# utcsilab/score-based-channels

Hardware: AMD Instinct MI355X
Metric: channels/s full ALD inference, CDL-C Nt64xNr16 (higher is better)
Workload: dtype f16x2 (every fp32 operand as two fp16 terms of a power-of-two-scaled value = 22-bit significand, hh + hl + lh on the fp16 matrix cores, fp32 accumulate; fp32-class by the gate tests/test_gpu_parity.py::test_f16x2_is_fp32_class and held to every reference golden at the north_star tolerance; unconditi

## Files before the change

### score_based_channels_amd/csrc/conv_down.hip

```cpp
#include <stdlib.h>
#include <string.h>
#include <type_traits>
#include "conv_common.h"

namespace sbc {

typedef float f32x4v __attribute__((ext_vector_type(4)));

struct DownParams {
    const float* __restrict__ a;
    const float* __restrict__ x;
    float* __restrict__ out;
    const float* __restrict__ stats;
    const uint4* __restrict__ w4;
    const uint4* __restrict__ w2;
    const float* __restrict__ bias;
    const float* __restrict__ bias2;
    unsigned* __restrict__ range_flag;
    float* __restrict__ calib;
    int B, H;
};

template <int B_, int E_, class F>
__device__ __forceinline__ void down_static_for(F&& f) {
    if constexpr (B_ < E_) {
        f(std::integral_constant<int, B_>{});
        down_static_for<B_ + 1, E_>(f);
    }
}

template <int CIN, int COUT, int W>
__global__ __launch_bounds__(256, 2) void conv_down_kernel(DownParams p) {
    constexpr int WO = W / 2, R = 8, NR = 2 * R + 2;
    constexpr int RP = W == 16 ? 12 : 6;
    constexpr int CG = CIN / 8, KH = CIN / 32, C4 = CIN / 4, NCB = COUT / 16;
    constexpr int NU = R * WO / 16;
    constexpr int RPU = 16 / WO;
    constexpr int PS = (2 * NR * RP * 16 + 255) / 256 * 256;
    constexpr int TERM = CG * PS;
    static_assert(NCB == 4, "four waves, one 16-output-channel block each");
    static_assert((W == 16 && CIN == 32) || (W == 8 && CIN == 64), "res2.0 (32 -> 64 at 16-pixel rows) and res3.0 (64 -> 64 at 8)");
    extern __shared__ __attribute__((aligned(256))) unsigned char smem[];

    const int tid = threadIdx.x, lane = tid & 63;
    const int cb = __builtin_amdgcn_readfirstlane(tid >> 6);
    const int kq = lane >> 4, n = lane & 15;
    const int H = p.H, HO = H / 2;
    const int tiles = HO / R;
    const int s = blockIdx.x / tiles, y0 = (blockIdx.x - s * tiles) * R;
    const int r_in0 = 2 * y0 - 1;

    const int wl_base = (((kq >> 1) * (COUT / 32) + (cb >> 1)) * 2) * 64 + (16 * (cb & 1) + n) + 32 * (kq & 1);
    constexpr int WD = 4;
    uint4 wr[WD][2];
    auto ldw = [&](const uint4* __restrict__ w, int tap, int kh, int slot) {
        const int idx = wl_base + ((tap * (CIN / 16) + 2 * kh) * (COUT / 32) * 2) * 64;
        wr[slot][0] = w[idx];
        wr[slot][1] = w[idx + 64];
    };
    const float4 tr4 = f16x2_trailer(reinterpret_cast<const float4*>(p.w4), 16 * (CIN / 16) * (COUT / 32) * 2);
    const float4 tr2 = f16x2_trailer(reinterpret_cast<const float4*>(p.w2), 4 * (CIN / 16) * (COUT / 32) * 2);
    const float scale_m = __builtin_bit_cast(float, __builtin_amdgcn_readfirstlane(__builtin_bit_cast(int, tr4.x)));
    const float scale_s = __builtin_bit_cast(float, __builtin_amdgcn_readfirstlane(__builtin_bit_cast(int, tr2.x)));
    const float descale_m = tr4.y, descale_s = tr2.y;
    const bool elu_acc = __builtin_amdgcn_readfirstlane(__builtin_bit_cast(int, tr4.w)) != 0;
    unsigned rbits = 0;

    const int c4 = tid % C4;
    constexpr int CPR = W * C4;
    auto plane_dst = [&](int prow, int col) {
        return smem + (c4 >> 1) * PS + (((col & 1) * NR + prow) * RP + (col >> 1) + (col & 1)) * 16 + (c4 & 1) * 8;
    };
    for (int i = tid; i < 2 * TERM / 16; i += 256) *reinterpret_cast<uint4*>(smem + i * 16) = make_uint4(0, 0, 0, 0);

    constexpr int NQA = NR * CPR / 256, NQX = 2 * R * CPR / 256;
    static_assert(NR * CPR % 256 == 0 && 2 * R * CPR % 256 == 0, "whole rounds of chunks");
    float4 va[NQA];
    const float* a_base = p.a + (size_t)s * H * W * CIN;
#pragma unroll
    for (int k = 0; k < NQA; ++k) {
        const int q = k * 256 + tid, prow = q / CPR;
        const int r = r_in0 + prow;
        va[k] = make_float4(0.f, 0.f, 0.f, 0.f);
        if (r >= 0 && r < H) va[k] = *reinterpret_cast<const float4*>(a_base + (size_t)r * W * CIN + (q - prow * CPR) * 4);
    }
    const float* st = p.stats + (size_t)s * 3 * CIN + c4 * 4;
    const float4 mu = *reinterpret_cast<const float4*>(st), sc = *reinterpret_cast<const float4*>(st + CIN),
                 sh = *reinterpret_cast<const float4*>(st + 2 * CIN);
    ldw(p.w4, 0, 0, 0);
    ldw(p.w4, 1 / KH, 1 % KH, 1);
    ldw(p.w4, 2 / KH, 2 % KH, 2);
    __syncthreads();
    float ta = 0.f;
#pragma unroll
    for (int k = 0; k < NQA; ++k) {
        const int q = k * 256 + tid, prow = q / CPR, col = (q - prow * CPR) / C4;
        const int r = r_in0 + prow;
        if (r < 0 || r >= H) continue;
        float4 v = va[k];
        v.x = fmaf(v.x - mu.x, sc.x, sh.x); v.y = fmaf(v.y - mu.y, sc.y, sh.y);
        v.z = fmaf(v.z - mu.z, sc.z, sh.z); v.w = fmaf(v.w - mu.w, sc.w, sh.w);
        v = elu4(v, elu_acc);
        StageScale ss{scale_m, ta};
        scale_track(v, &ss);
        ta = ss.amax;
        uint2 h, l;
        split_f16x2(v, scale_m, h, l);
        unsigned char* dst = plane_dst(prow, col);
        *reinterpret_cast<uint2*>(dst) = h;
        *reinterpret_cast<uint2*>(dst + TERM) = l;
    }
    pair_range_tile(ta, scale_m, rbits, p.calib);
    float4 vx[NQX];
    const float* x_base = p.x + ((size_t)s * H + 2 * y0) * W * CIN;
#pragma unroll
    for (int k = 0; k < NQX; ++k) vx[k] = *reinterpret_cast<const float4*>(x_base + (size_t)(k * 256 + tid) * 4);
    lds_barrier();

    const int yl0 = n / WO, xo = n % WO;
    const int rd_base = kq * PS + ((2 * yl0) * RP + xo) * 16;
    f32x4v accm[NU], accs[NU];
    auto kloop = [&](auto mainc, const uint4* __restrict__ w, f32x4v* acc) {
        constexpr bool MAIN = decltype(mainc)::value;
        constexpr int KT = MAIN ? 4 : 2, NS = KT * KT * KH;
        down_static_for<0, NS>([&](auto sc_) {
            constexpr int s_ = decltype(sc_)::value;
            constexpr int tap = s_ / KH, kh = s_ % KH, tp = tap / KT, tq = tap % KT;
            if constexpr (s_ + WD - 1 < NS) ldw(w, (s_ + WD - 1) / KH, (s_ + WD - 1) % KH, (s_ + WD - 1) % WD);
            const f16x8 wh = __builtin_bit_cast(f16x8, wr[s_ % WD][0]);
            const f16x8 wl = __builtin_bit_cast(f16x8, wr[s_ % WD][1]);
            constexpr int prow = MAIN ? tp : tp + 1, q = MAIN ? tq : tq + 1;
            constexpr int off = (4 * kh) * PS + ((((q + 1) & 1) * NR + prow) * RP + (q >> 1)) * 16;
            f16x8 xh[NU], xl[NU];
#pragma unroll
            for (int u = 0; u < NU; ++u) {
                xh[u] = *reinterpret_cast<const f16x8*>(smem + rd_base + off + (2 * u * RPU * RP) * 16);
                xl[u] = *reinterpret_cast<const f16x8*>(smem + rd_base + off + (2 * u * RPU * RP) * 16 + TERM);
            }
#pragma unroll
            for (int u = 0; u < NU; ++u) {
                const f32x4v z = s_ == 0 ? f32x4v{0.f, 0.f, 0.f, 0.f} : acc[u];
                acc[u] = __builtin_amdgcn_mfma_f32_16x16x32_f16(wh, xl[u], z, 0, 0, 0);
            }
#pragma unroll
            for (int u = 0; u < NU; ++u) acc[u] = __builtin_amdgcn_mfma_f32_16x16x32_f16(wl, xh[u], acc[u], 0, 0, 0);
#pragma unroll
            for (int u = 0; u < NU; ++u) acc[u] = __builtin_amdgcn_mfma_f32_16x16x32_f16(wh, xh[u], acc[u], 0, 0, 0);
            __builtin_amdgcn_sched_barrier(0);
        });
    };
    kloop(std::true_type{}, p.w4, accm);

    ldw(p.w2, 0, 0, 0);
    ldw(p.w2, 1 / KH, 1 % KH, 1);
    ldw(p.w2, 2 / KH, 2 % KH, 2);
    float tb = 0.f;
    uint2 xh_[NQX], xl_[NQX];
#pragma unroll
    for (int k = 0; k < NQX; ++k) {
        StageScale ss{scale_s, tb};
        scale_track(vx[k], &ss);
        tb = ss.amax;
        split_f16x2(vx[k], scale_s, xh_[k], xl_[k]);
    }
    pair_range_tile(tb, scale_s, rbits, p.calib ? p.calib + 1 : nullptr);
    lds_barrier();
#pragma unroll
    for (int k = 0; k < NQX; ++k) {
        const int q = k * 256 + tid, prow = q / CPR, col = (q - prow * CPR) / C4;
        unsigned char* dst = plane_dst(prow + 1, col);
        *reinterpret_cast<uint2*>(dst) = xh_[k];
        *reinterpret_cast<uint2*>(dst + TERM) = xl_[k];
    }
    lds_barrier();
    kloop(std::false_type{}, p.w2, accs);

    const int ch0 = 16 * cb + 4 * kq;
    const f32x4v b2 = *reinterpret_cast<const f32x4v*>(p.bias + ch0), bs = *reinterpret_cast<const f32x4v*>(p.bias2 + ch0);
#pragma unroll
    for (int u = 0; u < NU; ++u) {
        float4 o;
        o.x = fmaf(accs[u][0], descale_s, bs[0]) + fmaf(accm[u][0], descale_m, b2[0]);
        o.y = fmaf(accs[u][1], descale_s, bs[1]) + fmaf(accm[u][1], descale_m, b2[1]);
        o.z = fmaf(accs[u][2], descale_s, bs[2]) + fmaf(accm[u][2], descale_m, b2[2]);
        o.w = fmaf(accs[u][3], descale_s, bs[3]) + fmaf(accm[u][3], descale_m, b2[3]);
        const int y = y0 + u * RPU + yl0;
        st_out(p.out + (((size_t)s * HO + y) * WO + xo) * COUT + ch0, o);
    }
    if (rbits && lane == 0) atomicOr(p.range_flag, rbits);
}

template <int CIN, int COUT, int W>
static int launch_down_t(const DownParams& p, hipStream_t stream, bool dry) {
    constexpr int NR = 18, RP = W == 16 ? 12 : 6;
    constexpr int PS = (2 * NR * RP * 16 + 255) / 256 * 256;
    constexpr int LDS = 2 * (CIN / 8) * PS;
    auto kern = conv_down_kernel<CIN, COUT, W>;
    { const int rc = ensure_dyn_lds(reinterpret_cast<const void*>(kern), LDS); if (rc) return rc; }
    if (dry) return SBC_OK;
    hipLaunchKernelGGL(kern, dim3(p.B * (p.H / 2 / 8)), dim3(256), LDS, stream, p);
    SBC_CHECK_HIP(hipGetLastError());
    return SBC_OK;
}

int launch_conv_down(const sbc_op& op, hipStream_t stream, bool dry) {
    SBC_REQUIRE(op.in && op.out && op.res1 && op.stats && op.weight_split && op.weight2_split && op.bias && op.bias2,
                "conv_down: in / res1 / out / stats / weight_split / weight2_split / bias / bias2 must be set");
    SBC_REQUIRE((op.W == 16 && op.cin == 32 && op.cout == 64) || (op.W == 8 && op.cin == 64 && op.cout == 64),
                "conv_down: 32 -> 64 channels at 16-pixel rows or 64 -> 64 at 8 (got %d -> %d, W = %d)", op.cin, op.cout, op.W);
    SBC_REQUIRE(op.H % 16 == 0 && op.H >= 16, "conv_down: H = %d must be a multiple of 16 (tiles of 8 pooled rows)", op.H);
    SBC_REQUIRE((op.flags & SBC_CONV_F16X2) && !(op.flags & SBC_CONV_F16W), "conv_down: SBC_CONV_F16X2 only (the weight forms it reads)");
    SBC_REQUIRE(op.out != op.in && op.out != op.res1, "conv_down: out must not alias its inputs");
    SBC_REQUIRE(op.B > 0 && (long)op.B * op.H * op.W * op.cin <= 0x7fffffffL, "conv_down: bad batch %d", op.B);
    DownParams p;
    memset(&p, 0, sizeof(p));
    p.a = (const float*)op.in; p.x = (const float*)op.res1; p.out = (float*)op.out; p.stats = (const float*)op.stats;
    p.w4 = (const uint4*)op.weight_split; p.w2 = (const uint4*)op.weight2_split;
    p.bias = (const float*)op.bias; p.bias2 = (const float*)op.bias2;
    p.calib = (float*)op.calib;
    p.B = op.B; p.H = op.H;
    unsigned* flag = nullptr;
    { const int rc = range_flag_ptr(&flag); if (rc) return rc; }
    p.range_flag = flag;
    return op.W == 16 ? launch_down_t<32, 64, 16>(p, stream, dry) : launch_down_t<64, 64, 8>(p, stream, dry);
}

}
```

Baseline: 56.86.

## Make conv_down persistent with XCD-aware tiling and cross-tile prefetch

The down-sampling conv kernel now launches a persistent grid of about two workgroups per CU, grouped per XCD. Each workgroup walks a contiguous range of tiles and prefetches the next tile's activations, residual and stats while the current tile's MFMA loops run. The shortcut weights are held in registers for the whole kernel, and the LDS zero-fill happens once instead of per tile. This cuts launch/tail imbalance and global-load latency between tiles, at the cost of more register pressure, extra barriers per tile, and a hipDeviceGetAttribute query on every launch.

New measurement: 56.84 (median of 2 runs). No clear change (-0.0%).

```diff
diff --git a/score_based_channels_amd/csrc/conv_down.hip b/score_based_channels_amd/csrc/conv_down.hip
--- a/score_based_channels_amd/csrc/conv_down.hip
+++ b/score_based_channels_amd/csrc/conv_down.hip
@@ -19,6 +19,7 @@
     unsigned* __restrict__ range_flag;
     float* __restrict__ calib;
     int B, H;
+    int ntiles, tiles_per_xcd, wgs_per_xcd;
 };
 
 template <int B_, int E_, class F>
@@ -47,16 +48,25 @@
     const int kq = lane >> 4, n = lane & 15;
     const int H = p.H, HO = H / 2;
     const int tiles = HO / R;
-    const int s = blockIdx.x / tiles, y0 = (blockIdx.x - s * tiles) * R;
-    const int r_in0 = 2 * y0 - 1;
-
-    const int wl_base = (((kq >> 1) * (COUT / 32) + (cb >> 1)) * 2) * 64 + (16 * (cb & 1) + n) + 32 * (kq & 1);
+
+    const int xcd = blockIdx.x & 7, jw = blockIdx.x >> 3;
+    const int t_begin = xcd * p.tiles_per_xcd;
+    const int cnt = max(min(t_begin + p.tiles_per_xcd, p.ntiles) - t_begin, 0);
+    const int t0 = t_begin + jw * cnt / p.wgs_per_xcd, t1 = t_begin + (jw + 1) * cnt / p.wgs_per_xcd;
+    if (t0 >= t1) return;
+
+    auto opaque = [](int v) { asm volatile("" : "+v"(v)); return v; };
+    auto wl_base = [&](int l) { return ((((l >> 4) >> 1) * (COUT / 32) + (cb >> 1)) * 2) * 64 + (16 * (cb & 1) + (l & 15)) + 32 * ((l >> 4) & 1); };
     constexpr int WD = 4;
     uint4 wr[WD][2];
-    auto ldw = [&](const uint4* __restrict__ w, int tap, int kh, int slot) {
-        const int idx = wl_base + ((tap * (CIN / 16) + 2 * kh) * (COUT / 32) * 2) * 64;
-        wr[slot][0] = w[idx];
-        wr[slot][1] = w[idx + 64];
+    auto ldw = [&](const uint4* __restrict__ w, int wb, int tap, int kh, uint4* dst) {
+        const int idx = wb + ((tap * (CIN / 16) + 2 * kh) * (COUT / 32) * 2) * 64;
+        dst[0] = w[idx];
+        dst[1] = w[idx + 64];
+    };
+    auto ring_start = [&](const uint4* __restrict__ w) {
+        const int wb = wl_base(opaque(lane));
+        down_static_for<0, WD - 1>([&](auto sc_) { ldw(w, wb, decltype(sc_)::value / KH, decltype(sc_)::value % KH, wr[decltype(sc_)::value]); });
     };
     const float4 tr4 = f16x2_trailer(reinterpret_cast<const float4*>(p.w4), 16 * (CIN / 16) * (COUT / 32) * 2);
     const float4 tr2 = f16x2_trailer(reinterpret_cast<const float4*>(p.w2), 4 * (CIN / 16) * (COUT / 32) * 2);
@@ -65,70 +75,63 @@
     const float descale_m = tr4.y, descale_s = tr2.y;
     const bool elu_acc = __builtin_amdgcn_readfirstlane(__builtin_bit_cast(int, tr4.w)) != 0;
     unsigned rbits = 0;
-
-    const int c4 = tid % C4;
+    const int ch0 = 16 * cb + 4 * kq;
+    const f32x4v b2 = *reinterpret_cast<const f32x4v*>(p.bias + ch0), bs = *reinterpret_cast<const f32x4v*>(p.bias2 + ch0);
+    constexpr int NSS = 4 * KH;
+    uint4 ws[NSS][2];
+    down_static_for<0, NSS>([&](auto sc_) { ldw(p.w2, wl_base(lane), decltype(sc_)::value / KH, decltype(sc_)::value % KH, ws[decltype(sc_)::value]); });
+
     constexpr int CPR = W * C4;
-    auto plane_dst = [&](int prow, int col) {
+    auto plane_dst = [&](int tq, int prow, int col) {
+        const int c4 = tq % C4;
         return smem + (c4 >> 1) * PS + (((col & 1) * NR + prow) * RP + (col >> 1) + (col & 1)) * 16 + (c4 & 1) * 8;
     };
-    for (int i = tid; i < 2 * TERM / 16; i += 256) *reinterpret_cast<uint4*>(smem + i * 16) = make_uint4(0, 0, 0, 0);
-
     constexpr int NQA = NR * CPR / 256, NQX = 2 * R * CPR / 256;
     static_assert(NR * CPR % 256 == 0 && 2 * R * CPR % 256 == 0, "whole rounds of chunks");
-    float4 va[NQA];
-    const float* a_base = p.a + (size_t)s * H * W * CIN;
-#pragma unroll
-    for (int k = 0; k < NQA; ++k) {
-        const int q = k * 256 + tid, prow = q / CPR;
-        const int r = r_in0 + prow;
-        va[k] = make_float4(0.f, 0.f, 0.f, 0.f);
-        if (r >= 0 && r < H) va[k] = *reinterpret_cast<const float4*>(a_base + (size_t)r * W * CIN + (q - prow * CPR) * 4);
-    }
-    const float* st = p.stats + (size_t)s * 3 * CIN + c4 * 4;
-    const float4 mu = *reinterpret_cast<const float4*>(st), sc = *reinterpret_cast<const float4*>(st + CIN),
-                 sh = *reinterpret_cast<const float4*>(st + 2 * CIN);
-    ldw(p.w4, 0, 0, 0);
-    ldw(p.w4, 1 / KH, 1 % KH, 1);
-    ldw(p.w4, 2 / KH, 2 % KH, 2);
-    __syncthreads();
-    float ta = 0.f;
-#pragma unroll
-    for (int k = 0; k < NQA; ++k) {
-        const int q = k * 256 + tid, prow = q / CPR, col = (q - prow * CPR) / C4;
-        const int r = r_in0 + prow;
-        if (r < 0 || r >= H) continue;
-        float4 v = va[k];
-        v.x = fmaf(v.x - mu.x, sc.x, sh.x); v.y = fmaf(v.y - mu.y, sc.y, sh.y);
-        v.z = fmaf(v.z - mu.z, sc.z, sh.z); v.w = fmaf(v.w - mu.w, sc.w, sh.w);
-        v = elu4(v, elu_acc);
-        StageScale ss{scale_m, ta};
-        scale_track(v, &ss);
-        ta = ss.amax;
-        uint2 h, l;
-        split_f16x2(v, scale_m, h, l);
-        unsigned char* dst = plane_dst(prow, col);
-        *reinterpret_cast<uint2*>(dst) = h;
-        *reinterpret_cast<uint2*>(dst + TERM) = l;
-    }
-    pair_range_tile(ta, scale_m, rbits, p.calib);
-    float4 vx[NQX];
-    const float* x_base = p.x + ((size_t)s * H + 2 * y0) * W * CIN;
-#pragma unroll
-    for (int k = 0; k < NQX; ++k) vx[k] = *reinterpret_cast<const float4*>(x_base + (size_t)(k * 256 + tid) * 4);
+    float4 va[NQA], vx[NQX], mu, sc, sh;
+    auto request_a = [&](int s, int y0) {
+        const float* a_base = p.a + (size_t)s * H * W * CIN;
+        const int tq = opaque(tid);
+#pragma unroll
+        for (int k = 0; k < NQA; ++k) {
+            const int q = k * 256 + tq, prow = q / CPR;
+            const int r = min(max(2 * y0 - 1 + prow, 0), H - 1);
+            va[k] = *reinterpret_cast<const float4*>(a_base + (size_t)r * W * CIN + (q - prow * CPR) * 4);
+        }
+    };
+    auto request_x = [&](int s, int y0) {
+        const float* x_base = p.x + ((size_t)s * H + 2 * y0) * W * CIN;
+        const int tq = opaque(tid);
+#pragma unroll
+        for (int k = 0; k < NQX; ++k) vx[k] = *reinterpret_cast<const float4*>(x_base + (size_t)(k * 256 + tq) * 4);
+    };
+    auto request_stats = [&](int s) {
+        const float* st = p.stats + (size_t)s * 3 * CIN + (opaque(tid) % C4) * 4;
+        mu = *reinterpret_cast<const float4*>(st);
+        sc = *reinterpret_cast<const float4*>(st + CIN);
+        sh = *reinterpret_cast<const float4*>(st + 2 * CIN);
+    };
+
+    int s = t0 / tiles, j = t0 - s * tiles;
+    request_a(s, j * R);
+    request_stats(s);
+    ring_start(p.w4);
+    request_x(s, j * R);
+    for (int i = tid; i < 2 * TERM / 16; i += 256) *reinterpret_cast<uint4*>(smem + i * 16) = make_uint4(0, 0, 0, 0);
     lds_barrier();
 
     const int yl0 = n / WO, xo = n % WO;
     const int rd_base = kq * PS + ((2 * yl0) * RP + xo) * 16;
-    f32x4v accm[NU], accs[NU];
     auto kloop = [&](auto mainc, const uint4* __restrict__ w, f32x4v* acc) {
         constexpr bool MAIN = decltype(mainc)::value;
         constexpr int KT = MAIN ? 4 : 2, NS = KT * KT * KH;
+        const int wb = MAIN ? wl_base(opaque(lane)) : 0;
         down_static_for<0, NS>([&](auto sc_) {
             constexpr int s_ = decltype(sc_)::value;
             constexpr int tap = s_ / KH, kh = s_ % KH, tp = tap / KT, tq = tap % KT;
-            if constexpr (s_ + WD - 1 < NS) ldw(w, (s_ + WD - 1) / KH, (s_ + WD - 1) % KH, (s_ + WD - 1) % WD);
-            const f16x8 wh = __builtin_bit_cast(f16x8, wr[s_ % WD][0]);
-            const f16x8 wl = __builtin_bit_cast(f16x8, wr[s_ % WD][1]);
+            if constexpr (MAIN && s_ + WD - 1 < NS) ldw(w, wb, (s_ + WD - 1) / KH, (s_ + WD - 1) % KH, wr[(s_ + WD - 1) % WD]);
+            const f16x8 wh = __builtin_bit_cast(f16x8, MAIN ? wr[s_ % WD][0] : ws[MAIN ? 0 : s_][0]);
+            const f16x8 wl = __builtin_bit_cast(f16x8, MAIN ? wr[s_ % WD][1] : ws[MAIN ? 0 : s_][1]);
             constexpr int prow = MAIN ? tp : tp + 1, q = MAIN ? tq : tq + 1;
             constexpr int off = (4 * kh) * PS + ((((q + 1) & 1) * NR + prow) * RP + (q >> 1)) * 16;
             f16x8 xh[NU], xl[NU];
@@ -149,56 +152,95 @@
             __builtin_amdgcn_sched_barrier(0);
         });
     };
-    kloop(std::true_type{}, p.w4, accm);
-
-    ldw(p.w2, 0, 0, 0);
-    ldw(p.w2, 1 / KH, 1 % KH, 1);
-    ldw(p.w2, 2 / KH, 2 % KH, 2);
-    float tb = 0.f;
-    uint2 xh_[NQX], xl_[NQX];
-#pragma unroll
-    for (int k = 0; k < NQX; ++k) {
-        StageScale ss{scale_s, tb};
-        scale_track(vx[k], &ss);
-        tb = ss.amax;
-        split_f16x2(vx[k], scale_s, xh_[k], xl_[k]);
-    }
-    pair_range_tile(tb, scale_s, rbits, p.calib ? p.calib + 1 : nullptr);
-    lds_barrier();
-#pragma unroll
-    for (int k = 0; k < NQX; ++k) {
-        const int q = k * 256 + tid, prow = q / CPR, col = (q - prow * CPR) / C4;
-        unsigned char* dst = plane_dst(prow + 1, col);
-        *reinterpret_cast<uint2*>(dst) = xh_[k];
-        *reinterpret_cast<uint2*>(dst + TERM) = xl_[k];
-    }
-    lds_barrier();
-    kloop(std::false_type{}, p.w2, accs);
-
-    const int ch0 = 16 * cb + 4 * kq;
-    const f32x4v b2 = *reinterpret_cast<const f32x4v*>(p.bias + ch0), bs = *reinterpret_cast<const f32x4v*>(p.bias2 + ch0);
-#pragma unroll
-    for (int u = 0; u < NU; ++u) {
-        float4 o;
-        o.x = fmaf(accs[u][0], descale_s, bs[0]) + fmaf(accm[u][0], descale_m, b2[0]);
-        o.y = fmaf(accs[u][1], descale_s, bs[1]) + fmaf(accm[u][1], descale_m, b2[1]);
-        o.z = fmaf(accs[u][2], descale_s, bs[2]) + fmaf(accm[u][2], descale_m, b2[2]);
-        o.w = fmaf(accs[u][3], descale_s, bs[3]) + fmaf(accm[u][3], descale_m, b2[3]);
-        const int y = y0 + u * RPU + yl0;
-        st_out(p.out + (((size_t)s * HO + y) * WO + xo) * COUT + ch0, o);
+
+    for (int t = t0; t < t1; ++t) {
+        const int y0 = j * R, r_in0 = 2 * y0 - 1;
+        int s_nx = s, j_nx = j + 1;
+        if (j_nx == tiles) { j_nx = 0; ++s_nx; }
+        float ta = 0.f;
+        int tq = opaque(tid);
+#pragma unroll
+        for (int k = 0; k < NQA; ++k) {
+            const int q = k * 256 + tq, prow = q / CPR, col = (q - prow * CPR) / C4;
+            const int r = r_in0 + prow;
+            float4 v = va[k];
+            v.x = fmaf(v.x - mu.x, sc.x, sh.x); v.y = fmaf(v.y - mu.y, sc.y, sh.y);
+            v.z = fmaf(v.z - mu.z, sc.z, sh.z); v.w = fmaf(v.w - mu.w, sc.w, sh.w);
+            v = elu4(v, elu_acc);
+            if (r < 0 || r >= H) v = make_float4(0.f, 0.f, 0.f, 0.f);
+            StageScale ss{scale_m, ta};
+            scale_track(v, &ss);
+            ta = ss.amax;
+            uint2 h, l;
+            split_f16x2(v, scale_m, h, l);
+            unsigned char* dst = plane_dst(tq, prow, col);
+            *reinterpret_cast<uint2*>(dst) = h;
+            *reinterpret_cast<uint2*>(dst + TERM) = l;
+        }
+        pair_range_tile(ta, scale_m, rbits, p.calib);
+        lds_barrier();
+
+        f32x4v accm[NU], accs[NU];
+        kloop(std::true_type{}, p.w4, accm);
+
+        const bool more = t + 1 < t1;
+        ring_start(p.w4);
+        if (more) {
+            request_a(s_nx, j_nx * R);
+            if (s_nx != s) request_stats(s_nx);
+        }
+        lds_barrier();
+        float tb = 0.f;
+        tq = opaque(tid);
+#pragma unroll
+        for (int k = 0; k < NQX; ++k) {
+            const int q = k * 256 + tq, prow = q / CPR, col = (q - prow * CPR) / C4;
+            StageScale ss{scale_s, tb};
+            scale_track(vx[k], &ss);
+            tb = ss.amax;
+            uint2 h, l;
+            split_f16x2(vx[k], scale_s, h, l);
+            unsigned char* dst = plane_dst(tq, prow + 1, col);
+            *reinterpret_cast<uint2*>(dst) = h;
+            *reinterpret_cast<uint2*>(dst + TERM) = l;
+        }
+        pair_range_tile(tb, scale_s, rbits, p.calib ? p.calib + 1 : nullptr);
+        if (more) request_x(s_nx, j_nx * R);
+        lds_barrier();
+        kloop(std::false_type{}, p.w2, accs);
+
+#pragma unroll
+        for (int u = 0; u < NU; ++u) {
+            float4 o;
+            o.x = fmaf(accs[u][0], descale_s, bs[0]) + fmaf(accm[u][0], descale_m, b2[0]);
+            o.y = fmaf(accs[u][1], descale_s, bs[1]) + fmaf(accm[u][1], descale_m, b2[1]);
+            o.z = fmaf(accs[u][2], descale_s, bs[2]) + fmaf(accm[u][2], descale_m, b2[2]);
+            o.w = fmaf(accs[u][3], descale_s, bs[3]) + fmaf(accm[u][3], descale_m, b2[3]);
+            const int y = y0 + u * RPU + yl0;
+            st_out(p.out + (((size_t)s * HO + y) * WO + xo) * COUT + ch0, o);
+        }
+        lds_barrier();
+        s = s_nx; j = j_nx;
     }
     if (rbits && lane == 0) atomicOr(p.range_flag, rbits);
 }
 
 template <int CIN, int COUT, int W>
-static int launch_down_t(const DownParams& p, hipStream_t stream, bool dry) {
+static int launch_down_t(const DownParams& p0, hipStream_t stream, bool dry) {
     constexpr int NR = 18, RP = W == 16 ? 12 : 6;
     constexpr int PS = (2 * NR * RP * 16 + 255) / 256 * 256;
     constexpr int LDS = 2 * (CIN / 8) * PS;
     auto kern = conv_down_kernel<CIN, COUT, W>;
     { const int rc = ensure_dyn_lds(reinterpret_cast<const void*>(kern), LDS); if (rc) return rc; }
     if (dry) return SBC_OK;
-    hipLaunchKernelGGL(kern, dim3(p.B * (p.H / 2 / 8)), dim3(256), LDS, stream, p);
+    DownParams p = p0;
+    p.ntiles = p.B * (p.H / 2 / 8);
+    int dev = 0, cus = 256;
+    SBC_CHECK_HIP(hipGetDevice(&dev));
+    SBC_CHECK_HIP(hipDeviceGetAttribute(&cus, hipDeviceAttributeMultiprocessorCount, dev));
+    p.tiles_per_xcd = (p.ntiles + 7) / 8;
+    p.wgs_per_xcd = max(1, min(2 * persistent_cus(cus) / 8, p.tiles_per_xcd));
+    hipLaunchKernelGGL(kern, dim3(8 * p.wgs_per_xcd), dim3(256), LDS, stream, p);
     SBC_CHECK_HIP(hipGetLastError());
     return SBC_OK;
 }
```
